# jean-pierreBoth/gsearch

Hardware: AMD Instinct MI355X
Metric: query genomes/sec (higher is better)
Workload: dtype f32

## Files before the change

### gsearch_amd/csrc/gs_join.hip

```cpp
#include <string.h>
#include <algorithm>
#include <chrono>
#include <vector>
#include "gs_internal.hpp"

namespace gs {

template <typename T> struct ElemKey;
template <> struct ElemKey<uint32_t> { static constexpr bool F = false; };

template <int KIND, typename T>
__device__ __forceinline__ T canon(T v)
{
    if (KIND == GS_KIND_F32) return (v == (T)0x80000000u) ? (T)0 : v;
    return v;
}
template <int KIND, typename T>
__device__ __forceinline__ bool never_equal(T v)
{
    if (KIND == GS_KIND_F32) return ((uint32_t)v & 0x7FFFFFFFu) > 0x7F800000u;
    return false;
}

template <typename T>
__global__ __launch_bounds__(256) void k_rows_to_cols(const uint8_t *__restrict__ rows, uint64_t stride, uint64_t nrows, uint32_t m, T *__restrict__ cols,
                                                       uint64_t colcap, uint64_t first, int f32)
{
    __shared__ T tile[32][33];
    const uint32_t tx = threadIdx.x & 31, ty = threadIdx.x >> 5;
    const uint64_t r0 = (uint64_t)blockIdx.x * 32, s0 = (uint64_t)blockIdx.y * 32;
    for (uint32_t j = ty; j < 32; j += 8) {
        const uint64_t r = r0 + j, s = s0 + tx;
        tile[j][tx] = (r < nrows && s < m) ? ((const T *)(rows + r * stride))[s] : (T)0;
    }
    __syncthreads();
    for (uint32_t j = ty; j < 32; j += 8) {
        const uint64_t s = s0 + j, r = r0 + tx;
        if (s < m && r < nrows) { const T v = tile[tx][j]; cols[s * colcap + first + r] = (f32 && v == (T)0x80000000u) ? (T)0 : v; }
    }
}

template <int KIND, typename T>
__global__ __launch_bounds__(256) void k_query_cols(const uint8_t *__restrict__ rows, uint64_t stride, uint32_t nq, uint32_t m, T *__restrict__ qkey)
{
    __shared__ T tile[32][33];
    const uint32_t tx = threadIdx.x & 31, ty = threadIdx.x >> 5;
    const uint64_t r0 = (uint64_t)blockIdx.x * 32, s0 = (uint64_t)blockIdx.y * 32;
    for (uint32_t j = ty; j < 32; j += 8) {
        const uint64_t r = r0 + j, s = s0 + tx;
        tile[j][tx] = (r < nq && s < m) ? ((const T *)(rows + r * stride))[s] : (T)0;
    }
    __syncthreads();
    for (uint32_t j = ty; j < 32; j += 8) {
        const uint64_t s = s0 + j, r = r0 + tx;
        if (s < m && r < nq) qkey[s * nq + r] = tile[tx][j];
    }
}

constexpr int JT = 1024;
constexpr int JU = 4;
constexpr int JP_MAX_LOG2 = 13;
constexpr int JQ_MAX = 3276;
constexpr int JB_LOG2 = 16;
constexpr uint32_t HTILE = 128;

__device__ __forceinline__ uint32_t join_hash(uint32_t k) { return k * 0x9E3779B1u; }
__device__ __forceinline__ uint32_t join_hash(uint64_t k) { return (uint32_t)((k * 0x9E3779B97F4A7C15ull) >> 32); }
#define GS_SEL4(a, i) (((i) & 2) ? (((i) & 1) ? a[3] : a[2]) : (((i) & 1) ? a[1] : a[0]))

#ifndef GS_JOIN_COUNT_KIND
#define GS_JOIN_COUNT_KIND 0
#endif
constexpr int JN = 8;
__device__ __forceinline__ void join_lds_barrier()
{
    __builtin_amdgcn_fence(__ATOMIC_RELEASE, "workgroup", "local");
    __builtin_amdgcn_s_barrier();
    __builtin_amdgcn_fence(__ATOMIC_ACQUIRE, "workgroup", "local");
}

__device__ __forceinline__ void join_wave_sync()
{
    __builtin_amdgcn_fence(__ATOMIC_RELEASE, "wavefront");
    __builtin_amdgcn_wave_barrier();
    __builtin_amdgcn_fence(__ATOMIC_ACQUIRE, "wavefront");
}

#define GS_JOIN_HIT(st, tagv, e)                                                                              \
    do {                                                                                                      \
        if (((st) & 0xFFFu) == (tagv)) (st) += 0x1000u;                                                       \
        else if ((st) < 0x2000u) { if (st) { join_flush(mm32, ld, (st), (e)); natom++; } (st) = (tagv) | 0x1000u; } \
        else { join_flush(mm32, ld, (tagv) | 0x1000u, (e)); natom++; }                                        \
    } while (0)
__device__ __forceinline__ void join_flush(uint32_t *mm32, uint64_t ld, uint32_t st, uint64_t e)
{
    const uint64_t idx = (uint64_t)((st & 0xFFFu) - 1) * ld + e;
    atomicSub(&mm32[idx >> 1], (st >> 12) << ((idx & 1) * 16));
}

constexpr uint32_t JTAG_MASK = 0xFFFu, JTAG_MULTI = 0x1000u, JTAG_MORE = 0x80000000u;
constexpr int JTAG_CL_SHIFT = 13;
constexpr uint32_t JCL_MAX = 2047;
constexpr int JWALK = 4;

template <int KIND, typename T, int SR, bool CL>
__global__ __launch_bounds__(JT, (sizeof(T) == 8 && SR == 1) ? 4 : 8) void k_match_join(const T *__restrict__ qkey, uint32_t nq, uint32_t log2p, const T *__restrict__ cols, uint64_t colcap, uint64_t n,
                                                    uint32_t slot_lo, uint32_t slot_hi, uint32_t slots_per_wg, uint32_t *__restrict__ mm32, uint64_t ld,
                                                    unsigned long long *__restrict__ stats, int chunk_major, uint64_t col0, const uint16_t *__restrict__ qcl,
                                                    const uint16_t *__restrict__ nodelab, const T *__restrict__ qs, uint32_t nh, const uint32_t *__restrict__ cl_lo,
                                                    const uint32_t *__restrict__ qlist, uint32_t dedup_flags)
{
    const uint32_t dedup_below = dedup_flags & 0x7FFFFFFFu;
    static_assert(JU == 4 && JN % JU == 0, "GS_SEL4 / pending mask are written for JU = 4");
    static_assert(!CL || SR == 1, "clusters: request batches only");
    constexpr bool E8 = sizeof(T) == 4 && SR == 1;
    constexpr bool DEDUP = CL && E8;
    constexpr bool D64 = sizeof(T) == 8 && SR == 1 && !CL;
    constexpr bool DENSE = E8 || D64;
    extern __shared__ __attribute__((aligned(16))) uint8_t s_raw[];
    const uint32_t P = 1u << log2p, mask = P - 1, sh = 32 - log2p;
    constexpr uint32_t BMW = (1u << JB_LOG2) / 32;
    uint32_t *tag = (uint32_t *)s_raw;
    uint32_t *bm = E8 ? (uint32_t *)(s_raw + 8 * (size_t)P) : (uint32_t *)(s_raw + 4 * (size_t)P * SR);
    T *key = (T *)(s_raw + (4 * (size_t)P + (size_t)BMW * 4) * SR);
    unsigned long long *ent = (unsigned long long *)s_raw;
    const uint32_t bchunk = chunk_major ? blockIdx.y : blockIdx.x, bslot = chunk_major ? blockIdx.x : blockIdx.y;
    const uint64_t e0 = (uint64_t)bchunk * (JT * JN) + threadIdx.x;
    const uint32_t s0 = slot_lo + bslot * slots_per_wg, s1 = s0 + slots_per_wg < slot_hi ? s0 + slots_per_wg : slot_hi;
    const uint2 *labT = CL ? (const uint2 *)nodelab + (uint64_t)bchunk * (JN / JU) * JT : nullptr;
    uint32_t sticky[JN];
    uint32_t natom = 0;
    uint32_t nexp = 0;
#pragma unroll
    for (int i = 0; i < JN; i++) sticky[i] = 0;
    const uint32_t lane = threadIdx.x & 63;
    uint32_t vmask = 0;
#pragma unroll
    for (int u = 0; u < JN; u++) vmask |= (uint32_t)(e0 + (uint64_t)u * JT < n) << u;
    const uint64_t ebase_u = col0 + (uint64_t)bchunk * (JT * JN);
    const uint32_t tid = threadIdx.x;
    uint32_t labmask = 0;
    if (CL && DENSE) {
#pragma unroll
        for (int it = 0; it < JN / JU; it++) {
            const uint2 l4 = labT[it * JT + threadIdx.x];
            labmask |= ((uint32_t)((l4.x & 0xFFFFu) != 0u) | (uint32_t)((l4.x >> 16) != 0u) << 1 | (uint32_t)((l4.y & 0xFFFFu) != 0u) << 2 | (uint32_t)((l4.y >> 16) != 0u) << 3) << (it * JU);
        }
    }
    const bool wave_lab = CL && DENSE && (dedup_flags >> 31) && __any(labmask != 0u);
    uint2 *wq = (uint2 *)(s_raw + (D64 ? 12 : 8) * (size_t)P + (size_t)BMW * 4) + (threadIdx.x >> 6) * (D64 ? 128 : 64);
    T vn[DENSE ? JN : JU];
#pragma unroll
    for (int u = 0; u < (DENSE ? JN : JU); u++) { const uint64_t e = e0 + (uint64_t)u * JT; vn[u] = (e < n && s0 < s1) ? cols[(uint64_t)s0 * colcap + e] : (T)0; }
    for (uint32_t sr = s0; sr < s1; sr += SR) {
        const uint32_t nr = s1 - sr < (uint32_t)SR ? s1 - sr : (uint32_t)SR;
        constexpr int JQ = DENSE ? (int)((((1u << JP_MAX_LOG2) * 2) / 5 + JT - 1) / JT) : 1;
        T kq[JQ];
        uint32_t tq[(JQ + 1) / 2] = {};
        if (DENSE) {
            typedef const T __attribute__((address_space(1))) *gptr;
            const uint64_t qb = (uint64_t)(qkey + (uint64_t)sr * nq);
            const gptr qk = (gptr)(((uint64_t)(uint32_t)__builtin_amdgcn_readfirstlane((uint32_t)(qb >> 32)) << 32) | (uint64_t)(uint32_t)__builtin_amdgcn_readfirstlane((uint32_t)qb));
            uint32_t o = threadIdx.x;
            asm volatile("" : "+v"(o));
#pragma unroll
            for (int j = 0; j < JQ; j++) { const gptr qj = qk + j * JT; kq[j] = o + (uint32_t)j * JT < nq ? qj[o] : (T)0; }
            if constexpr (CL) {
#pragma unroll
                for (int j = 0; j < JQ; j++) { const uint32_t i = o + (uint32_t)j * JT; tq[j >> 1] |= (i < nq ? (uint32_t)qcl[i] : 0u) << ((j & 1) * 16); }
            }
        }
        join_lds_barrier();
        if (E8) { for (uint32_t i = threadIdx.x; i < P; i += JT) ent[i] = 0ull; }
        else for (uint32_t i = threadIdx.x; i < P * SR; i += JT) tag[i] = 0;
        for (uint32_t i = threadIdx.x; i < BMW * SR; i += JT) bm[i] = 0;
        join_lds_barrier();
        auto insert_key = [&](const uint32_t r, const uint32_t q, T k, const uint32_t clq) {
            const uint32_t tw = CL ? (q + 1) | (clq << JTAG_CL_SHIFT) : q + 1;
            if (never_equal<KIND, T>(k)) return;
            k = canon<KIND, T>(k);
            const uint32_t hq = join_hash(k);
            atomicOr(&bm[r * BMW + (hq >> (32 - JB_LOG2 + 5))], (1u << ((hq >> (32 - JB_LOG2)) & 31)) | (1u << ((hq >> (27 - JB_LOG2)) & 31)));
            uint32_t h = hq >> sh;
            if (E8) {
                const unsigned long long nw = ((unsigned long long)tw << 32) | (uint32_t)k;
                for (;;) {
                    const unsigned long long old = atomicCAS(&ent[h], 0ull, nw);
                    if (old == 0ull) break;
                    if (DEDUP && (tw >> JTAG_CL_SHIFT) - 1u < dedup_below - 1u && (uint32_t)old == (uint32_t)k &&
                        (((uint32_t)(old >> 32) >> JTAG_CL_SHIFT) & JCL_MAX) == (tw >> JTAG_CL_SHIFT)) {
                        atomicOr((uint32_t *)&ent[h] + 1, JTAG_MULTI);
                        break;
                    }
                    if ((uint32_t)old == (uint32_t)k && !((uint32_t)(old >> 32) & JTAG_MORE)) atomicOr((uint32_t *)&ent[h] + 1, JTAG_MORE);
                    h = (h + 1) & mask;
                }
            } else {
                while (atomicCAS(&tag[r * P + h], 0u, tw) != 0u) h = (h + 1) & mask;
                key[r * P + h] = k;
            }
        };
        if (DENSE) {
#pragma unroll
            for (int j = 0; j < JQ; j++) { const uint32_t i = threadIdx.x + (uint32_t)j * JT; if (i < nq) insert_key(0u, i, kq[j], (tq[j >> 1] >> ((j & 1) * 16)) & 0xFFFFu); }
        } else {
            for (uint32_t i = threadIdx.x; i < nq * nr; i += JT) { const uint32_t r = i / nq, q = i - r * nq; insert_key(r, q, qkey[(uint64_t)(sr + r) * nq + q], CL ? (uint32_t)qcl[q] : 0u); }
        }
        uint2 lb0 = make_uint2(0u, 0u), lb1 = make_uint2(0u, 0u);
        if constexpr (CL && DENSE) {
            if (wave_lab) { uint32_t o0 = threadIdx.x, o1 = JT + threadIdx.x; asm volatile("" : "+v"(o0), "+v"(o1)); lb0 = labT[o0]; lb1 = labT[o1]; }
        }
        join_lds_barrier();
#pragma unroll 1
        for (uint32_t r = 0; r < nr; r++) {
            const uint32_t s = sr + r, tb = r * P, bb = r * BMW;
            const T *col = cols + (uint64_t)s * colcap;
            if constexpr (DENSE) {
                uint32_t pend = 0;
#pragma unroll
                for (int u0 = 0; u0 < JN; u0 += 4) {
                    uint32_t hsd[4], bwd[4];
#pragma unroll
                    for (int u = 0; u < 4; u++) { hsd[u] = join_hash(vn[u0 + u]); bwd[u] = bm[hsd[u] >> (32 - JB_LOG2 + 5)]; }
#pragma unroll
                    for (int u = 0; u < 4; u++) {
                        const uint32_t pass = (vmask >> (u0 + u)) & (bwd[u] >> ((hsd[u] >> (32 - JB_LOG2)) & 31)) & (bwd[u] >> ((hsd[u] >> (27 - JB_LOG2)) & 31)) & 1u;
                        pend |= pass << (u0 + u);
                    }
                }
                if constexpr (CL) {
                    if (wave_lab) {
#pragma unroll
                        for (int u = 0; u < JN; u++) {
                            const uint32_t l2 = u < 4 ? ((u & 2) ? lb0.y : lb0.x) : ((u & 2) ? lb1.y : lb1.x);
                            const uint32_t lab = (l2 >> ((u & 1) * 16)) & 0xFFFFu;
                            if (((pend >> u) & 1u) && lab != 0u) {
                                uint32_t hh = join_hash(vn[u]) >> sh;
#pragma unroll
                                for (int j = 0; j < JWALK; j++) {
                                    const unsigned long long en = ent[hh];
                                    const uint32_t t = (uint32_t)(en >> 32);
                                    if (t == 0u) { pend &= ~(1u << u); natom += GS_JOIN_COUNT_KIND == 8; break; }
                                    if ((uint32_t)en == (uint32_t)vn[u]) {
                                        if (((t >> JTAG_CL_SHIFT) & JCL_MAX) != lab) break;
                                        if (!(t & JTAG_MORE)) { pend &= ~(1u << u); natom += GS_JOIN_COUNT_KIND == 8; break; }
                                    }
                                    hh = (hh + 1) & mask;
                                }
                            }
                        }
                    }
                }
                while (__any(pend != 0u)) {
                    uint32_t qn = 0;
                    const uint32_t pend0 = pend;
#pragma unroll
                    for (int u = 0; u < JN; u++) {
                        const bool want = (pend >> u) & 1u;
                        const unsigned long long mw = __ballot(want);
                        const uint32_t cw = (uint32_t)__popcll(mw);
                        if (cw != 0u && qn + cw <= 64u) {
                            if (want) {
                                const uint32_t at = qn + __builtin_amdgcn_mbcnt_hi((uint32_t)(mw >> 32), __builtin_amdgcn_mbcnt_lo((uint32_t)mw, 0u));
                                const uint32_t who = lane | ((uint32_t)u << 6) | (sticky[u] << 9) | (CL ? ((labmask >> u) & 1u) << 29 : 0u);
                                if constexpr (D64) { wq[2 * at] = make_uint2((uint32_t)vn[u], (uint32_t)((uint64_t)vn[u] >> 32)); wq[2 * at + 1].x = who; }
                                else wq[at] = make_uint2((uint32_t)vn[u], who);
                            }
                            qn += cw; pend &= ~(1u << u);
                        }
                    }
                    join_wave_sync();
                    if constexpr (CL) {
                        if (GS_JOIN_COUNT_KIND == 7 && lane < qn) natom++;
                        bool have = lane < qn;
                        uint2 qe = make_uint2(0u, 0u);
                        if (have) qe = wq[lane];
                        uint32_t st = (qe.y >> 9) & 0xFFFFFu, flp = 0;
                        const uint32_t eloc = (qe.y & 63u) + ((qe.y >> 6) & 7u) * JT;
                        uint32_t hh = join_hash((T)qe.x) >> sh;
                        for (;;) {
                            uint32_t mitem = 0;
                            if (have) {
                                const unsigned long long en = ent[hh];
                                const uint32_t t = (uint32_t)(en >> 32);
                                if (t == 0u) have = false;
                                else {
                                    if ((uint32_t)en == qe.x) {
                                        if (!(t & JTAG_MORE)) have = false;
                                        bool count_it = true;
// ... 249 lines not shown
    __shared__ uint2 stage[HS_STAGE];
    __shared__ uint32_t sn;
    __shared__ unsigned long long sbase;
    if (threadIdx.x == 0) sn = 0;
    __syncthreads();
    const uint64_t tiles_per_row = (n + 2047) / 2048, ntiles = tiles_per_row * nq;
    uint32_t tot = 0;
    auto flush = [&]() {
        __syncthreads();
        const uint32_t cnt = sn;
        if (cnt) {
            if (threadIdx.x == 0) sbase = atomicAdd(&ctr[0], (unsigned long long)cnt);
            __syncthreads();
            const unsigned long long base = sbase;
            for (uint32_t i = threadIdx.x; i < cnt; i += 256) if (base + i < cap) pairs[base + i] = stage[i];
            __syncthreads();
            if (threadIdx.x == 0) sn = 0;
        }
        __syncthreads();
    };
    for (uint64_t t = blockIdx.x; t < ntiles; t += gridDim.x) {
        const uint32_t q = (uint32_t)(t / tiles_per_row);
        const uint64_t e8 = (t - (uint64_t)q * tiles_per_row) * 2048 + (uint64_t)threadIdx.x * 8;
        if (e8 < n) {
            const uint4 w = *(const uint4 *)(mat + (uint64_t)q * ld + e8);
            const uint32_t ww[4] = {w.x, w.y, w.z, w.w};
#pragma unroll
            for (int i = 0; i < 8; i++) {
                const uint32_t c = (ww[i >> 1] >> ((i & 1) * 16)) & 0xFFFFu;
                const uint32_t def = (e8 + i < n) ? m - c : 0u;
                tot += def;
                if (def >= JHEAVY) stage[atomicAdd(&sn, 1u)] = make_uint2((uint32_t)(e8 + i), q | (def << 16));
            }
        }
        __syncthreads();
        if (sn >= HS_STAGE - 2048) flush();
    }
    flush();
#pragma unroll
    for (int o = 32; o > 0; o >>= 1) tot += __shfl_down(tot, o);
    if ((threadIdx.x & 63) == 0 && tot) atomicAdd(&ctr[1], (unsigned long long)tot);
}
__global__ void k_label_init(uint32_t *__restrict__ labq, uint32_t nq, uint32_t *__restrict__ labe, uint64_t n)
{
    const uint64_t i = (uint64_t)blockIdx.x * blockDim.x + threadIdx.x;
    if (i < nq) labq[i] = (uint32_t)i;
    if (i < n) labe[i] = 0xFFFFFFFFu;
}
__global__ void k_label_prop(const uint2 *__restrict__ pairs, const unsigned long long *__restrict__ ctr, uint64_t cap, uint32_t *__restrict__ labq, uint32_t *__restrict__ labe)
{
    const uint64_t np = ctr[0] < cap ? ctr[0] : cap;
    for (uint64_t i = (uint64_t)blockIdx.x * blockDim.x + threadIdx.x; i < np; i += (uint64_t)gridDim.x * blockDim.x) {
        const uint2 p = pairs[i];
        const uint32_t q = p.y & 0xFFFFu, a = labq[q], b = labe[p.x], l = a < b ? a : b;
        if (l < a) atomicMin(&labq[q], l);
        if (l < b) atomicMin(&labe[p.x], l);
    }
}
__global__ void k_label_count(const uint32_t *__restrict__ labe, uint64_t n, uint32_t nq, uint32_t *__restrict__ cnt)
{
    for (uint64_t e = (uint64_t)blockIdx.x * blockDim.x + threadIdx.x; e < n; e += (uint64_t)gridDim.x * blockDim.x) { const uint32_t l = labe[e]; if (l < nq) atomicAdd(&cnt[l], 1u); }
}
template <typename T>
__global__ __launch_bounds__(256) void k_query_cols_list(const uint8_t *__restrict__ rows, uint64_t stride, const uint32_t *__restrict__ qlist, uint32_t nh, uint32_t m, T *__restrict__ qs)
{
    __shared__ T tile[32][33];
    const uint32_t tx = threadIdx.x & 31, ty = threadIdx.x >> 5;
    const uint64_t r0 = (uint64_t)blockIdx.x * 32, s0 = (uint64_t)blockIdx.y * 32;
    for (uint32_t j = ty; j < 32; j += 8) {
        const uint64_t r = r0 + j, s = s0 + tx;
        tile[j][tx] = (r < nh && s < m) ? ((const T *)(rows + (uint64_t)qlist[r] * stride))[s] : (T)0;
    }
    __syncthreads();
    for (uint32_t j = ty; j < 32; j += 8) {
        const uint64_t s = s0 + j, r = r0 + tx;
        if (s < m && r < nh) qs[s * nh + r] = tile[tx][j];
    }
}
struct JoinGeom { uint32_t chunks, log2p; size_t lds1, ldsq; };

template <int KIND, typename T, bool CL>
static int join_launch(gs_ctx *c, const JoinGeom &g, const T *qkey, uint32_t nq, const void *cols, uint64_t colcap, uint64_t n, uint32_t slot_lo, uint32_t slot_hi,
                       uint16_t *out16, uint64_t ld, unsigned long long *stats, uint64_t col0, bool few_blocks, const uint16_t *qcl, const uint16_t *nodelab, const T *qs,
                       uint32_t nh, const uint32_t *cl_lo, const uint32_t *qlist, uint32_t dedup_below = 0)
{
    const uint32_t ms = slot_hi - slot_lo, chunks = g.chunks;
    uint32_t blocks = std::max<uint32_t>(1, std::min<uint32_t>((16 * c->n_cu) / chunks, std::max<uint32_t>(ms / 32, (2 * c->n_cu) / chunks)));
    if (few_blocks) blocks = std::max<uint32_t>(1, std::min<uint32_t>(ms / 4, (2 * c->n_cu + chunks - 1) / chunks));
    if (getenv("GS_JOIN_BLOCKS") && !few_blocks) blocks = (uint32_t)atoi(getenv("GS_JOIN_BLOCKS"));
    blocks = std::min<uint32_t>(std::max<uint32_t>(blocks, 1), ms);
    const uint32_t slots_per_wg = (ms + blocks - 1) / blocks;
    const int chunk_major = getenv("GS_JOIN_CHUNK_MAJOR") ? atoi(getenv("GS_JOIN_CHUNK_MAJOR")) : ((nq >= 1024 && chunks >= 16) ? 1 : 0);
    const uint32_t nblk = (ms + slots_per_wg - 1) / slots_per_wg;
    dim3 jg(chunk_major ? nblk : chunks, chunk_major ? chunks : nblk);
    int sr = 1;
    if (!CL) {
        if (4 * g.lds1 <= 80 * 1024 && slots_per_wg >= 8) sr = 4; else if (2 * g.lds1 <= 80 * 1024 && slots_per_wg >= 4) sr = 2;
        if (getenv("GS_JOIN_SLOTS_PER_ROUND")) { const int e = atoi(getenv("GS_JOIN_SLOTS_PER_ROUND")); if (e == 1 || (e == 2 && 2 * g.lds1 <= 80 * 1024) || (e == 4 && 4 * g.lds1 <= 80 * 1024)) sr = e; }
    }
    const size_t lds = g.lds1 * sr + (sr == 1 ? g.ldsq : 0);
    ProfScope ps(c, FAM_HAMMING);
#define GS_JOIN_GO(KERN)                                                                                                                              \
    do {                                                                                                                                              \
        auto kern = KERN;                                                                                                                             \
        if (lds > 48 * 1024) GS_HIP_CHECK(hipFuncSetAttribute((const void *)kern, hipFuncAttributeMaxDynamicSharedMemorySize, (int)lds));             \
        hipLaunchKernelGGL(kern, jg, dim3(JT), lds, c->stream, qkey, nq, g.log2p, (const T *)cols, colcap, n, slot_lo, slot_hi, slots_per_wg, (uint32_t *)out16, ld, \
                           stats, chunk_major, col0, qcl, nodelab, qs, nh, cl_lo, qlist, dedup_below);                                                             \
    } while (0)
    if (CL) GS_JOIN_GO((k_match_join<KIND, T, 1, CL>));
    else if (sr == 4) GS_JOIN_GO((k_match_join<KIND, T, 4, false>));
    else if (sr == 2) GS_JOIN_GO((k_match_join<KIND, T, 2, false>));
    else GS_JOIN_GO((k_match_join<KIND, T, 1, false>));
#undef GS_JOIN_GO
    GS_HIP_CHECK(hipGetLastError());
    return GS_OK;
}

template <int KIND, typename T>
static int join_sample_declines(gs_ctx *c, const JoinGeom &g, uint32_t m, const T *qkey, uint32_t nq, const void *cols, uint64_t colcap, uint64_t n, DevBuf *scratch, int *decline_out)
{
    int rc;
    const uint32_t nsamp = 24;
    DevBuf &cnt = scratch[1];
    if ((rc = cnt.ensure(16))) return rc;
    GS_HIP_CHECK(hipMemsetAsync(cnt.p, 0, 16, c->stream));
    const size_t lds_s = (sizeof(T) + 4) * ((size_t)1 << g.log2p);
    auto ks = k_match_sample<KIND, T>;
    if (lds_s > 48 * 1024) GS_HIP_CHECK(hipFuncSetAttribute((const void *)ks, hipFuncAttributeMaxDynamicSharedMemorySize, (int)lds_s));
    hipLaunchKernelGGL(ks, dim3(g.chunks, nsamp), dim3(JT), lds_s, c->stream, qkey, nq, g.log2p, (const T *)cols, colcap, n, m, nsamp, cnt.as<unsigned long long>());
    GS_HIP_CHECK(hipGetLastError());
    unsigned long long hr[2] = {0, 0};
    GS_HIP_CHECK(hipMemcpyAsync(hr, cnt.p, 16, hipMemcpyDeviceToHost, c->stream));
    GS_HIP_CHECK(hipStreamSynchronize(c->stream));
    const double scale = (double)m / (double)nsamp;
    const double atomics = (double)(hr[0] - hr[1]) * scale + (double)hr[1] * scale / 64.0;
    const double t_join = (double)n * m * sizeof(T) / 3.5e12 + atomics / 1.6e10 + (double)hr[0] * scale / 2.0e11;
    const double t_tile = (double)((nq + 127) / 128 * 128) * (double)n * (double)m / (KIND == GS_KIND_U64 ? 1.4e13 : 1.6e13);
    const char *force = getenv("GS_JOIN_DECLINE");
    const bool decline = force ? atoi(force) != 0 : t_join > t_tile;
    if (getenv("GS_JOIN_VERBOSE"))
        fprintf(stderr, "[GS_JOIN] nq=%u n=%llu sampled matches %llu repeats %llu -> est. join %.2f ms, tile %.2f ms: %s\n", nq, (unsigned long long)n, hr[0], hr[1],
                t_join * 1e3, t_tile * 1e3, decline ? "tile" : "join");
    *decline_out = decline ? 1 : 0;
    return GS_OK;
}

template <int KIND, typename T>
static int join_impl(gs_ctx *c, uint32_t m, const uint8_t *qrows, uint64_t qstride, uint32_t nq, const void *cols, uint64_t colcap, uint64_t n, uint16_t *out16,
                     uint64_t ld, DevBuf *scratch , int *declined, unsigned long long *stats, bool init, uint64_t col0,
                     const void *rows, uint64_t rstride)
{
    int rc;
    if (declined) *declined = 0;
    const size_t items = (size_t)m * nq;
    DevBuf &k0 = scratch[0];
    if ((rc = k0.ensure(sizeof(T) * items))) return rc;
    if (init) GS_HIP_CHECK(hipMemsetD16Async((hipDeviceptr_t)out16, (unsigned short)m, (size_t)nq * ld, c->stream));
    dim3 tg((nq + 31) / 32, (m + 31) / 32);
    hipLaunchKernelGGL((k_query_cols<KIND, T>), tg, dim3(256), 0, c->stream, qrows, qstride, nq, m, k0.as<T>());
    GS_HIP_CHECK(hipGetLastError());
    JoinGeom g;
    g.log2p = 6;
    while (g.log2p < (uint32_t)JP_MAX_LOG2 && (double)(1u << g.log2p) * 0.4 < (double)nq) g.log2p++;
    g.chunks = (uint32_t)((n + (uint64_t)JT * JN - 1) / ((uint64_t)JT * JN));
    g.lds1 = (sizeof(T) + 4) * ((size_t)1 << g.log2p) + ((size_t)1 << JB_LOG2) / 8;
    g.ldsq = (size_t)(JT / 64) * 64 * (sizeof(T) == 4 ? 8 : 16);
    const bool may_decline = declined && m >= 64 && n >= 4096;
    const char *ce = getenv("GS_JOIN_CLUSTER");
    bool cluster = declined && init && col0 == 0 && rows && nq >= 256 && n >= 8192 && m >= 16 * JS0 && (ld % 8) == 0 && !(ce && !atoi(ce)) && !getenv("GS_JOIN_DECLINE");
    if (ce && atoi(ce) == 2) cluster = declined && init && col0 == 0 && rows && m >= 2 * JS0 && (ld % 8) == 0;
    if (!cluster) {
        if (may_decline) {
            int dec = 0;
            if ((rc = join_sample_declines<KIND, T>(c, g, m, k0.as<T>(), nq, cols, colcap, n, scratch, &dec))) return rc;
            if (dec) { *declined = 1; return GS_OK; }
        }
        return join_launch<KIND, T, false>(c, g, k0.as<T>(), nq, cols, colcap, n, 0, m, out16, ld, stats, col0, false, nullptr, nullptr, nullptr, 0, nullptr, nullptr);
    }
    const bool verbose = getenv("GS_JOIN_VERBOSE") != nullptr;
    const bool times = getenv("GS_JOIN_TIMES") != nullptr;
    auto t_prev = std::chrono::steady_clock::now();
    auto lap = [&](const char *what) {
        if (!times) return;
        (void)hipStreamSynchronize(c->stream);
        const auto now = std::chrono::steady_clock::now();
        fprintf(stderr, "[GS_JOIN_TIMES] %-28s %8.3f ms\n", what, std::chrono::duration<double, std::milli>(now - t_prev).count());
        t_prev = now;
    };
    lap("query columns + memset");
    DevBuf &pairs = scratch[2], &ctr = scratch[3], &labq = scratch[4], &labe = scratch[5];
    uint64_t pair_cap = JPAIR_CAP;
    DevBuf &lcnt = scratch[14];
    if ((rc = pairs.ensure(pair_cap * 8)) || (rc = ctr.ensure(64)) || (rc = labq.ensure(4 * (size_t)nq)) || (rc = labe.ensure(4 * (size_t)n)) || (rc = lcnt.ensure(4 * (size_t)nq))) return rc;
    pair_cap = std::max<uint64_t>(pair_cap, pairs.bytes / 8);
    if ((rc = join_launch<KIND, T, false>(c, g, k0.as<T>(), nq, cols, colcap, n, 0, JS0, out16, ld, stats, 0, true, nullptr, nullptr, nullptr, 0, nullptr, nullptr))) return rc;
    lap("phase 0 (first slots)");
    uint8_t *pin = (uint8_t *)pinned_pool(c)->ensure(PIN_JOIN, 64 + 4 * (2 * (size_t)nq + n) + 2 * ((size_t)nq + 8 + (size_t)g.chunks * JT * JN) + 64);
    GS_REQUIRE(pin, GS_ERR_HIP, "match-join: pinned staging buffer");
    unsigned long long *hc = (unsigned long long *)pin;
    uint32_t *hlq = (uint32_t *)(pin + 64), *hcn = hlq + nq, *hle = hcn + nq;
    for (int attempt = 0;; attempt++) {
        GS_HIP_CHECK(hipMemsetAsync(ctr.p, 0, 64, c->stream));
        hipLaunchKernelGGL(k_heavy_scan, dim3(c->n_cu * 8), dim3(256), 0, c->stream, out16, ld, nq, n, m, pairs.as<uint2>(), ctr.as<unsigned long long>(), pair_cap);
        lap("heavy scan");
        hipLaunchKernelGGL(k_label_init, dim3((uint32_t)((std::max<uint64_t>(n, nq) + 255) / 256)), dim3(256), 0, c->stream, labq.as<uint32_t>(), nq, labe.as<uint32_t>(), n);
        for (int it = 0; it < 6; it++)
            hipLaunchKernelGGL(k_label_prop, dim3(c->n_cu * 4), dim3(256), 0, c->stream, pairs.as<uint2>(), ctr.as<unsigned long long>(), pair_cap, labq.as<uint32_t>(), labe.as<uint32_t>());
        GS_HIP_CHECK(hipMemsetAsync(lcnt.p, 0, 4 * (size_t)nq, c->stream));
        hipLaunchKernelGGL(k_label_count, dim3(c->n_cu * 2), dim3(256), 0, c->stream, labe.as<uint32_t>(), n, nq, lcnt.as<uint32_t>());
        GS_HIP_CHECK(hipGetLastError());
        GS_HIP_CHECK(hipMemcpyAsync(hc, ctr.p, 16, hipMemcpyDeviceToHost, c->stream));
        GS_HIP_CHECK(hipMemcpyAsync(hlq, labq.p, 4 * (size_t)nq, hipMemcpyDeviceToHost, c->stream));
        GS_HIP_CHECK(hipMemcpyAsync(hcn, lcnt.p, 4 * (size_t)nq, hipMemcpyDeviceToHost, c->stream));
        GS_HIP_CHECK(hipStreamSynchronize(c->stream));
        lap("labels + query labels down");
        if (hc[0] <= pair_cap || attempt || hc[0] > JPAIR_MAX) break;
        if (pairs.alloc((size_t)hc[0] * 8 + 4096) != GS_OK) { (void)hipGetLastError(); (void)pairs.alloc(JPAIR_CAP * 8); pair_cap = JPAIR_CAP; break; }
        pair_cap = hc[0] + 512;
    }
    const uint64_t npairs = hc[0];
    std::vector<uint32_t> cq(nq, 0), ce_(nq, 0), cid(nq, 0);
    uint32_t K = 0, ntiles = 0, nhq = 0, dedup_below = 1;
    uint64_t nhe = 0;
    const uint32_t minq = getenv("GS_JOIN_CLUSTER_MINQ") ? (uint32_t)std::max(2, atoi(getenv("GS_JOIN_CLUSTER_MINQ"))) : (ce && atoi(ce) == 2 ? 2u : 12u);
    const uint64_t minpairs = getenv("GS_JOIN_CLUSTER_MINPAIRS") ? (uint64_t)atoll(getenv("GS_JOIN_CLUSTER_MINPAIRS")) : 128;
    auto is_cluster = [&](uint32_t l) { return cq[l] >= minq || (cq[l] >= 2 && (uint64_t)(cq[l] - 1) * hcn[l] >= minpairs); };
    const uint64_t min_scaled0 = (uint64_t)((double)nq * 32.0 * (double)n / 3.0e5);
    const uint64_t min_saved0 = getenv("GS_JOIN_CLUSTER_MIN") ? (uint64_t)atoll(getenv("GS_JOIN_CLUSTER_MIN")) : (ce && atoi(ce) == 2 ? 0 : std::max<uint64_t>((uint64_t)nq * 8, min_scaled0));
    bool any = false;
    if (npairs <= pair_cap) {
        for (uint32_t q = 0; q < nq; q++) if (hlq[q] < nq) ++cq[hlq[q]];
        uint64_t est = 0;
        for (uint32_t l = 0; l < nq; l++) if (cq[l] && hcn[l] && is_cluster(l)) { any = true; est += (uint64_t)(cq[l] - 1) * hcn[l]; }
        if (est < min_saved0) any = false;
    }
    if (any) {
        GS_HIP_CHECK(hipMemcpyAsync(hle, labe.p, 4 * (size_t)n, hipMemcpyDeviceToHost, c->stream));
        GS_HIP_CHECK(hipStreamSynchronize(c->stream));
        for (uint64_t e = 0; e < n; e++) if (hle[e] < nq) ce_[hle[e]]++;
        std::vector<uint32_t> order;
        for (uint32_t l = 0; l < nq; l++) if (ce_[l] >= 1 && is_cluster(l)) order.push_back(l);
        auto tiles_of = [&](uint32_t l) { return ((cq[l] + HTILE - 1) / HTILE) * ((ce_[l] + HTILE - 1) / HTILE); };
        std::sort(order.begin(), order.end(), [&](uint32_t a, uint32_t b) { const uint32_t ta = tiles_of(a), tb = tiles_of(b); return ta != tb ? ta < tb : a < b; });
        std::vector<uint32_t> chosen;
        for (uint32_t l : order) {
            if (chosen.size() >= JCL_MAX || ntiles + tiles_of(l) > JTILE_CAP) break;
            chosen.push_back(l); ntiles += tiles_of(l); nhq += cq[l]; nhe += ce_[l];
        }
        const uint32_t dq = getenv("GS_JOIN_DEDUP_MINQ") ? (uint32_t)std::max(2, atoi(getenv("GS_JOIN_DEDUP_MINQ"))) : JDEDUP_MINQ;
        std::stable_sort(chosen.begin(), chosen.end(), [&](uint32_t a, uint32_t b) { return (cq[a] >= dq) > (cq[b] >= dq); });
        for (uint32_t l : chosen) { cid[l] = ++K; if (cq[l] >= dq) dedup_below = K + 1; }
    }
    uint64_t saved_pairs = 0;
    for (uint32_t l = 0; l < nq; l++) if (cid[l]) saved_pairs += (uint64_t)(cq[l] - 1) * ce_[l];
    const uint64_t min_scaled = (uint64_t)((double)nq * 32.0 * (double)n / 3.0e5);
    const uint64_t min_saved = getenv("GS_JOIN_CLUSTER_MIN") ? (uint64_t)atoll(getenv("GS_JOIN_CLUSTER_MIN")) : (ce && atoi(ce) == 2 ? 0 : std::max<uint64_t>((uint64_t)nq * 8, min_scaled));
    if (verbose)
        fprintf(stderr, "[GS_JOIN] nq=%u n=%llu heavy pairs %llu (matches in the first %u slots %llu): %u clusters, %u queries x %llu nodes in %u tiles, %llu pairs off the atomics%s\n", nq,
                (unsigned long long)n, (unsigned long long)npairs, JS0, hc[1], K, nhq, (unsigned long long)nhe, ntiles, (unsigned long long)saved_pairs,
                K && saved_pairs < min_saved ? " - not worth the cluster-aware pass" : "");
    if (K && saved_pairs < min_saved) K = 0;
    lap("host: components");
    if (K == 0) {
        const double t_tile = (double)((nq + 127) / 128 * 128) * (double)n * (double)m / (KIND == GS_KIND_U64 ? 1.4e13 : 1.6e13);
        if (may_decline && (npairs > pair_cap || (double)hc[1] * ((double)m / JS0) / 1.6e10 > 0.5 * t_tile)) {
            int dec = 0;
            if ((rc = join_sample_declines<KIND, T>(c, g, m, k0.as<T>(), nq, cols, colcap, n, scratch, &dec))) return rc;
            if (dec) { *declined = 1; return GS_OK; }
        }
        return join_launch<KIND, T, false>(c, g, k0.as<T>(), nq, cols, colcap, n, JS0, m, out16, ld, stats, 0, false, nullptr, nullptr, nullptr, 0, nullptr, nullptr);
    }
    std::vector<uint32_t> cl_lo(K + 2, 0), ce_lo(K + 2, 0);
    for (uint32_t l = 0; l < nq; l++) if (cid[l]) { cl_lo[cid[l] + 1] = cq[l]; ce_lo[cid[l] + 1] = ce_[l]; }
    for (uint32_t k = 1; k <= K + 1; k++) { cl_lo[k] += cl_lo[k - 1]; ce_lo[k] += ce_lo[k - 1]; }
    std::vector<uint32_t> qlist(nhq), elist(nhe), fq(cl_lo.begin(), cl_lo.end()), fe(ce_lo.begin(), ce_lo.end());
    const uint64_t npad = (uint64_t)g.chunks * JT * JN;
    uint16_t *hqcl = (uint16_t *)(hle + n), *hnl = hqcl + ((nq + 3) & ~3u);
    for (uint32_t q = 0; q < nq; q++) { const uint32_t l = hlq[q]; hqcl[q] = 0; if (l < nq && cid[l]) { hqcl[q] = (uint16_t)cid[l]; qlist[fq[cid[l]]++] = q; } }
    memset(hnl, 0, 2 * npad);
    for (uint64_t e = 0; e < n; e++) {
        const uint32_t l = hle[e];
        if (l < nq && cid[l]) {
            const uint64_t ch = e / (JT * JN), w = e % (JT * JN), i = w / JT, ln = w % JT;
            hnl[((ch * (JN / JU) + i / JU) * JT + ln) * JU + i % JU] = (uint16_t)cid[l];
            elist[fe[cid[l]]++] = (uint32_t)e;
        }
    }
    std::vector<uint4> tiles;
    tiles.reserve(ntiles);
    uint32_t n_thin = 0;
    for (int pass = 0; pass < 2; pass++)
        for (uint32_t k = 1; k <= K; k++)
            for (uint32_t a = cl_lo[k]; a < cl_lo[k + 1]; a += HTILE) {
                const uint32_t qr = std::min<uint32_t>(HTILE, cl_lo[k + 1] - a);
                if ((qr <= 16) != (pass == 0)) continue;
                for (uint32_t b = ce_lo[k]; b < ce_lo[k + 1]; b += HTILE) {
                    tiles.push_back(make_uint4(a, qr, b, std::min<uint32_t>(HTILE, ce_lo[k + 1] - b)));
                    n_thin += pass == 0;
                }
            }
    lap("host: lists");
    DevBuf &dqcl = scratch[6], &dnl = scratch[7], &dql = scratch[8], &del = scratch[9], &dtl = scratch[10], &dqs = scratch[11], &dcl = scratch[13];
    if ((rc = dqcl.ensure(2 * (size_t)nq)) || (rc = dnl.ensure(2 * (size_t)npad)) || (rc = dql.ensure(4 * (size_t)nhq)) || (rc = del.ensure(4 * (size_t)nhe)) ||
        (rc = dtl.ensure(16 * tiles.size())) || (rc = dqs.ensure(sizeof(T) * (size_t)m * nhq)) || (rc = dcl.ensure(4 * (size_t)(K + 2)))) return rc;
    GS_HIP_CHECK(hipMemcpyAsync(dqcl.p, hqcl, 2 * (size_t)nq, hipMemcpyHostToDevice, c->stream));
    GS_HIP_CHECK(hipMemcpyAsync(dnl.p, hnl, 2 * (size_t)npad, hipMemcpyHostToDevice, c->stream));
    GS_HIP_CHECK(hipMemcpyAsync(dql.p, qlist.data(), 4 * (size_t)nhq, hipMemcpyHostToDevice, c->stream));
    GS_HIP_CHECK(hipMemcpyAsync(del.p, elist.data(), 4 * (size_t)nhe, hipMemcpyHostToDevice, c->stream));
    GS_HIP_CHECK(hipMemcpyAsync(dtl.p, tiles.data(), 16 * tiles.size(), hipMemcpyHostToDevice, c->stream));
    GS_HIP_CHECK(hipMemcpyAsync(dcl.p, cl_lo.data(), 4 * (size_t)(K + 2), hipMemcpyHostToDevice, c->stream));
    GS_HIP_CHECK(hipStreamSynchronize(c->stream));
    hipLaunchKernelGGL((k_query_cols_list<T>), dim3((nhq + 31) / 32, (m + 31) / 32), dim3(256), 0, c->stream, qrows, qstride, dql.as<uint32_t>(), nhq, m, dqs.as<T>());
    GS_HIP_CHECK(hipGetLastError());
    lap("uploads + sorted key copy");
    const bool inplace = getenv("GS_JOIN_INPLACE") ? atoi(getenv("GS_JOIN_INPLACE")) != 0 : nhe * 10 >= n;
    if ((rc = join_launch<KIND, T, true>(c, g, k0.as<T>(), nq, cols, colcap, n, JS0, m, out16, ld, stats, 0, false, dqcl.as<uint16_t>(), dnl.as<uint16_t>(), dqs.as<T>(), nhq,
                                         dcl.as<uint32_t>(), dql.as<uint32_t>(), dedup_below | (inplace ? 0x80000000u : 0u)))) return rc;
    {
        ProfScope ps(c, FAM_HAMMING);
        lap("cluster-aware join");
        if ((rc = hamming_blocks(c, KIND, m, qrows, qstride, rows, rstride, dtl.p, (uint32_t)tiles.size(), dql.as<uint32_t>(), del.as<uint32_t>(), out16, ld, n_thin))) return rc;
        lap("block compare");
    }
    return GS_OK;
}

uint64_t match_join_max_queries() { const char *e = getenv("GS_JOIN_MAXQ"); return e ? (uint64_t)std::max(1, std::min(4094, atoi(e))) : JQ_MAX; }

int match_join_counts(gs_ctx *c, int kind, uint32_t m, const void *qrows, uint64_t qstride, uint64_t nq, const void *cols, uint64_t colcap, uint64_t n,
                      uint16_t *out16, uint64_t ld, DevBuf *scratch, int *declined, unsigned long long *stats, bool init, uint64_t col0, const void *rows, uint64_t rstride)
{
    GS_REQUIRE(nq >= 1 && nq <= 4094 && m <= 65535 && (ld % 2) == 0 && ((uintptr_t)out16 % 4) == 0, GS_ERR_INVALID, "match_join_counts: bad shape");
    GS_REQUIRE((uint64_t)m * nq < ((uint64_t)1 << 31), GS_ERR_INVALID, "match_join_counts: batch too large");
    if (kind == GS_KIND_U64) return join_impl<GS_KIND_U64, uint64_t>(c, m, (const uint8_t *)qrows, qstride, (uint32_t)nq, cols, colcap, n, out16, ld, scratch, declined, stats, init, col0, rows, rstride);
    if (kind == GS_KIND_F32) return join_impl<GS_KIND_F32, uint32_t>(c, m, (const uint8_t *)qrows, qstride, (uint32_t)nq, cols, colcap, n, out16, ld, scratch, declined, stats, init, col0, rows, rstride);
    return join_impl<GS_KIND_U32, uint32_t>(c, m, (const uint8_t *)qrows, qstride, (uint32_t)nq, cols, colcap, n, out16, ld, scratch, declined, stats, init, col0, rows, rstride);
}

int rows_to_cols(gs_ctx *c, int kind, uint32_t m, const void *rows, uint64_t stride, uint64_t nrows, void *cols, uint64_t colcap, uint64_t first)
{
    if (nrows == 0) return GS_OK;
    dim3 g((uint32_t)((nrows + 31) / 32), (m + 31) / 32);
    if (kind == GS_KIND_U64) hipLaunchKernelGGL((k_rows_to_cols<uint64_t>), g, dim3(256), 0, c->stream, (const uint8_t *)rows, stride, nrows, m, (uint64_t *)cols, colcap, first, 0);
    else hipLaunchKernelGGL((k_rows_to_cols<uint32_t>), g, dim3(256), 0, c->stream, (const uint8_t *)rows, stride, nrows, m, (uint32_t *)cols, colcap, first, (int)(kind == GS_KIND_F32));
    GS_HIP_CHECK(hipGetLastError());
    return GS_OK;
}

}
```

Measured before the change: 48390.

## Prebuild per-slot LDS hash table images once, load them in join

Adds a prepass kernel that builds each slot's query hash table and bloom bitmap once, then writes a compact image of entry positions and bitmap words to global memory. The f32 join kernel then loads these images and places entries directly into LDS instead of redoing atomic CAS inserts in every workgroup that shares the slot. This removes redundant per-chunk table construction and its atomic contention. The cost is an extra kernel launch, a global image buffer of slots×nq×8 bytes plus bitmaps, and extra global reads per slot.

```diff
diff --git a/gsearch_amd/csrc/gs_join.hip b/gsearch_amd/csrc/gs_join.hip
--- a/gsearch_amd/csrc/gs_join.hip
+++ b/gsearch_amd/csrc/gs_join.hip
@@ -103,18 +103,81 @@
 constexpr uint32_t JCL_MAX = 2047;
 constexpr int JWALK = 4;
 
+constexpr int JQ4 = (int)((((1u << JP_MAX_LOG2) * 2) / 5 + JT - 1) / JT);
+constexpr uint32_t JIMG_POS_HI = 1u << 24, JIMG_VALID = 1u << 25, JIMG_NONE = 0xFFFFFFFFu;
+constexpr uint32_t JIMG_TAG_KEEP = JTAG_MORE | JTAG_MULTI | (JCL_MAX << JTAG_CL_SHIFT);
+static_assert(JQ4 == 4 && JP_MAX_LOG2 == 13 && (JIMG_TAG_KEEP & (JTAG_MASK | JIMG_POS_HI | JIMG_VALID)) == 0, "image layout");
+static_assert((1u << JB_LOG2) / 32 == 2 * JT, "a lane copies two bitmap words");
+
+template <int KIND, bool CL>
+__device__ __forceinline__ uint32_t join_insert8(unsigned long long *ent, uint32_t *bm, uint32_t mask, uint32_t sh, uint32_t k, uint32_t q, uint32_t clq, uint32_t dedup_below)
+{
+    const uint32_t tw = CL ? (q + 1) | (clq << JTAG_CL_SHIFT) : q + 1;
+    if (never_equal<KIND, uint32_t>(k)) return JIMG_NONE;
+    k = canon<KIND, uint32_t>(k);
+    const uint32_t hq = join_hash(k);
+    atomicOr(&bm[hq >> (32 - JB_LOG2 + 5)], (1u << ((hq >> (32 - JB_LOG2)) & 31)) | (1u << ((hq >> (27 - JB_LOG2)) & 31)));
+    uint32_t h = hq >> sh;
+    const unsigned long long nw = ((unsigned long long)tw << 32) | k;
+    for (;;) {
+        const unsigned long long old = atomicCAS(&ent[h], 0ull, nw);
+        if (old == 0ull) return h;
+        if (CL && (tw >> JTAG_CL_SHIFT) - 1u < dedup_below - 1u && (uint32_t)old == k && (((uint32_t)(old >> 32) >> JTAG_CL_SHIFT) & JCL_MAX) == (tw >> JTAG_CL_SHIFT)) {
+            atomicOr((uint32_t *)&ent[h] + 1, JTAG_MULTI);
+            return JIMG_NONE;
+        }
+        if ((uint32_t)old == k && !((uint32_t)(old >> 32) & JTAG_MORE)) atomicOr((uint32_t *)&ent[h] + 1, JTAG_MORE);
+        h = (h + 1) & mask;
+    }
+}
+
+template <int KIND, bool CL>
+__global__ __launch_bounds__(JT) void k_join_tables(const uint32_t *__restrict__ qkey, uint32_t nq, uint32_t log2p, uint32_t slot_lo, const uint16_t *__restrict__ qcl, uint32_t dedup_below,
+                                                     unsigned long long *__restrict__ img_e, uint32_t *__restrict__ img_b)
+{
+    extern __shared__ __attribute__((aligned(16))) uint8_t s_raw[];
+    const uint32_t P = 1u << log2p, mask = P - 1, sh = 32 - log2p;
+    constexpr uint32_t BMW = (1u << JB_LOG2) / 32;
+    unsigned long long *ent = (unsigned long long *)s_raw;
+    uint32_t *bm = (uint32_t *)(s_raw + 8 * (size_t)P);
+    const uint32_t b = blockIdx.x;
+    const uint32_t *qk = qkey + (uint64_t)(slot_lo + b) * nq;
+    for (uint32_t i = threadIdx.x; i < P; i += JT) ent[i] = 0ull;
+    for (uint32_t i = threadIdx.x; i < BMW; i += JT) bm[i] = 0;
+    __syncthreads();
+    uint32_t at[JQ4];
+#pragma unroll
+    for (int j = 0; j < JQ4; j++) {
+        const uint32_t q = threadIdx.x + (uint32_t)j * JT;
+        at[j] = q < nq ? join_insert8<KIND, CL>(ent, bm, mask, sh, qk[q], q, CL ? (uint32_t)qcl[q] : 0u, dedup_below) : JIMG_NONE;
+    }
+    __syncthreads();
+#pragma unroll
+    for (int j = 0; j < JQ4; j++) {
+        const uint32_t q = threadIdx.x + (uint32_t)j * JT;
+        if (q < nq) {
+            unsigned long long e = 0ull;
+            if (at[j] != JIMG_NONE) {
+                const unsigned long long f = ent[at[j]];
+                e = (unsigned long long)(((uint32_t)(f >> 32) & JIMG_TAG_KEEP) | (at[j] & JTAG_MASK) | ((at[j] >> 12) << 24) | JIMG_VALID) << 32 | (uint32_t)f;
+            }
+            img_e[(uint64_t)b * nq + q] = e;
+        }
+    }
+    for (uint32_t i = threadIdx.x; i < BMW; i += JT) img_b[(uint64_t)b * BMW + i] = bm[i];
+}
+
 template <int KIND, typename T, int SR, bool CL>
 __global__ __launch_bounds__(JT, (sizeof(T) == 8 && SR == 1) ? 4 : 8) void k_match_join(const T *__restrict__ qkey, uint32_t nq, uint32_t log2p, const T *__restrict__ cols, uint64_t colcap, uint64_t n,
                                                     uint32_t slot_lo, uint32_t slot_hi, uint32_t slots_per_wg, uint32_t *__restrict__ mm32, uint64_t ld,
                                                     unsigned long long *__restrict__ stats, int chunk_major, uint64_t col0, const uint16_t *__restrict__ qcl,
                                                     const uint16_t *__restrict__ nodelab, const T *__restrict__ qs, uint32_t nh, const uint32_t *__restrict__ cl_lo,
-                                                    const uint32_t *__restrict__ qlist, uint32_t dedup_flags)
-{
-    const uint32_t dedup_below = dedup_flags & 0x7FFFFFFFu;
+                                                    const uint32_t *__restrict__ qlist, uint32_t dedup_flags, const unsigned long long *__restrict__ img_e,
+                                                    const uint32_t *__restrict__ img_b)
+{
     static_assert(JU == 4 && JN % JU == 0, "GS_SEL4 / pending mask are written for JU = 4");
     static_assert(!CL || SR == 1, "clusters: request batches only");
     constexpr bool E8 = sizeof(T) == 4 && SR == 1;
-    constexpr bool DEDUP = CL && E8;
     constexpr bool D64 = sizeof(T) == 8 && SR == 1 && !CL;
     constexpr bool DENSE = E8 || D64;
     extern __shared__ __attribute__((aligned(16))) uint8_t s_raw[];
@@ -154,10 +217,23 @@
     for (int u = 0; u < (DENSE ? JN : JU); u++) { const uint64_t e = e0 + (uint64_t)u * JT; vn[u] = (e < n && s0 < s1) ? cols[(uint64_t)s0 * colcap + e] : (T)0; }
     for (uint32_t sr = s0; sr < s1; sr += SR) {
         const uint32_t nr = s1 - sr < (uint32_t)SR ? s1 - sr : (uint32_t)SR;
-        constexpr int JQ = DENSE ? (int)((((1u << JP_MAX_LOG2) * 2) / 5 + JT - 1) / JT) : 1;
-        T kq[JQ];
-        uint32_t tq[(JQ + 1) / 2] = {};
-        if (DENSE) {
+        constexpr int JQ = DENSE ? JQ4 : 1;
+        T kq[E8 ? 1 : JQ];
+        unsigned long long ie[E8 ? JQ : 1];
+        unsigned long long ib = 0ull;
+        uint32_t o8 = 0;
+        if constexpr (E8) {
+            typedef const uint8_t __attribute__((address_space(1))) *gptr1;
+            typedef const unsigned long long __attribute__((address_space(1))) *gptr8;
+            const uint64_t qb = (uint64_t)(img_e + (uint64_t)(sr - slot_lo) * nq), bb = (uint64_t)((const uint2 *)img_b + (uint64_t)(sr - slot_lo) * JT);
+            const gptr1 qk = (gptr1)(((uint64_t)(uint32_t)__builtin_amdgcn_readfirstlane((uint32_t)(qb >> 32)) << 32) | (uint64_t)(uint32_t)__builtin_amdgcn_readfirstlane((uint32_t)qb));
+            const gptr1 bk = (gptr1)(((uint64_t)(uint32_t)__builtin_amdgcn_readfirstlane((uint32_t)(bb >> 32)) << 32) | (uint64_t)(uint32_t)__builtin_amdgcn_readfirstlane((uint32_t)bb));
+            o8 = threadIdx.x * 8u;
+            asm volatile("" : "+v"(o8));
+#pragma unroll
+            for (int j = 0; j < JQ; j++) ie[j] = threadIdx.x + (uint32_t)j * JT < nq ? *(gptr8)(qk + j * JT * 8 + o8) : 0ull;
+            ib = *(gptr8)(bk + o8);
+        } else if constexpr (DENSE) {
             typedef const T __attribute__((address_space(1))) *gptr;
             const uint64_t qb = (uint64_t)(qkey + (uint64_t)sr * nq);
             const gptr qk = (gptr)(((uint64_t)(uint32_t)__builtin_amdgcn_readfirstlane((uint32_t)(qb >> 32)) << 32) | (uint64_t)(uint32_t)__builtin_amdgcn_readfirstlane((uint32_t)qb));
@@ -165,46 +241,42 @@
             asm volatile("" : "+v"(o));
 #pragma unroll
             for (int j = 0; j < JQ; j++) { const gptr qj = qk + j * JT; kq[j] = o + (uint32_t)j * JT < nq ? qj[o] : (T)0; }
-            if constexpr (CL) {
-#pragma unroll
-                for (int j = 0; j < JQ; j++) { const uint32_t i = o + (uint32_t)j * JT; tq[j >> 1] |= (i < nq ? (uint32_t)qcl[i] : 0u) << ((j & 1) * 16); }
+        }
+        join_lds_barrier();
+        if constexpr (E8) {
+            if (log2p == (uint32_t)JP_MAX_LOG2) {
+#pragma unroll
+                for (int k = 0; k < 4; k++) *(uint4 *)(s_raw + k * 16 * JT + 2 * o8) = make_uint4(0u, 0u, 0u, 0u);
+            } else
+                for (uint32_t i = o8; i < 8 * P; i += 8 * JT) *(unsigned long long *)(s_raw + i) = 0ull;
+            join_lds_barrier();
+            *(unsigned long long *)((uint8_t *)bm + o8) = ib;
+#pragma unroll
+            for (int j = 0; j < JQ; j++) {
+                const uint32_t w = (uint32_t)(ie[j] >> 32);
+                if (w != 0u)
+                    ent[((w & JTAG_MASK) | ((w >> 12) & 0x1000u)) & mask] = (unsigned long long)((w & JIMG_TAG_KEEP) | (tid + (uint32_t)j * JT + 1u)) << 32 | (uint32_t)ie[j];
             }
-        }
-        join_lds_barrier();
-        if (E8) { for (uint32_t i = threadIdx.x; i < P; i += JT) ent[i] = 0ull; }
-        else for (uint32_t i = threadIdx.x; i < P * SR; i += JT) tag[i] = 0;
-        for (uint32_t i = threadIdx.x; i < BMW * SR; i += JT) bm[i] = 0;
-        join_lds_barrier();
-        auto insert_key = [&](const uint32_t r, const uint32_t q, T k, const uint32_t clq) {
-            const uint32_t tw = CL ? (q + 1) | (clq << JTAG_CL_SHIFT) : q + 1;
-            if (never_equal<KIND, T>(k)) return;
-            k = canon<KIND, T>(k);
-            const uint32_t hq = join_hash(k);
-            atomicOr(&bm[r * BMW + (hq >> (32 - JB_LOG2 + 5))], (1u << ((hq >> (32 - JB_LOG2)) & 31)) | (1u << ((hq >> (27 - JB_LOG2)) & 31)));
-            uint32_t h = hq >> sh;
-            if (E8) {
-                const unsigned long long nw = ((unsigned long long)tw << 32) | (uint32_t)k;
-                for (;;) {
-                    const unsigned long long old = atomicCAS(&ent[h], 0ull, nw);
-                    if (old == 0ull) break;
-                    if (DEDUP && (tw >> JTAG_CL_SHIFT) - 1u < dedup_below - 1u && (uint32_t)old == (uint32_t)k &&
-                        (((uint32_t)(old >> 32) >> JTAG_CL_SHIFT) & JCL_MAX) == (tw >> JTAG_CL_SHIFT)) {
-                        atomicOr((uint32_t *)&ent[h] + 1, JTAG_MULTI);
-                        break;
-                    }
-                    if ((uint32_t)old == (uint32_t)k && !((uint32_t)(old >> 32) & JTAG_MORE)) atomicOr((uint32_t *)&ent[h] + 1, JTAG_MORE);
-                    h = (h + 1) & mask;
-                }
-            } else {
+        } else {
+            for (uint32_t i = threadIdx.x; i < P * SR; i += JT) tag[i] = 0;
+            for (uint32_t i = threadIdx.x; i < BMW * SR; i += JT) bm[i] = 0;
+            join_lds_barrier();
+            auto insert_key = [&](const uint32_t r, const uint32_t q, T k, const uint32_t clq) {
+                const uint32_t tw = CL ? (q + 1) | (clq << JTAG_CL_SHIFT) : q + 1;
+                if (never_equal<KIND, T>(k)) return;
+                k = canon<KIND, T>(k);
+                const uint32_t hq = join_hash(k);
+                atomicOr(&bm[r * BMW + (hq >> (32 - JB_LOG2 + 5))], (1u << ((hq >> (32 - JB_LOG2)) & 31)) | (1u << ((hq >> (27 - JB_LOG2)) & 31)));
+                uint32_t h = hq >> sh;
                 while (atomicCAS(&tag[r * P + h], 0u, tw) != 0u) h = (h + 1) & mask;
                 key[r * P + h] = k;
+            };
+            if (DENSE) {
+#pragma unroll
+                for (int j = 0; j < JQ; j++) { const uint32_t i = threadIdx.x + (uint32_t)j * JT; if (i < nq) insert_key(0u, i, kq[j], 0u); }
+            } else {
+                for (uint32_t i = threadIdx.x; i < nq * nr; i += JT) { const uint32_t r = i / nq, q = i - r * nq; insert_key(r, q, qkey[(uint64_t)(sr + r) * nq + q], CL ? (uint32_t)qcl[q] : 0u); }
             }
-        };
-        if (DENSE) {
-#pragma unroll
-            for (int j = 0; j < JQ; j++) { const uint32_t i = threadIdx.x + (uint32_t)j * JT; if (i < nq) insert_key(0u, i, kq[j], (tq[j >> 1] >> ((j & 1) * 16)) & 0xFFFFu); }
-        } else {
-            for (uint32_t i = threadIdx.x; i < nq * nr; i += JT) { const uint32_t r = i / nq, q = i - r * nq; insert_key(r, q, qkey[(uint64_t)(sr + r) * nq + q], CL ? (uint32_t)qcl[q] : 0u); }
         }
         uint2 lb0 = make_uint2(0u, 0u), lb1 = make_uint2(0u, 0u);
         if constexpr (CL && DENSE) {
@@ -620,7 +692,7 @@
 template <int KIND, typename T, bool CL>
 static int join_launch(gs_ctx *c, const JoinGeom &g, const T *qkey, uint32_t nq, const void *cols, uint64_t colcap, uint64_t n, uint32_t slot_lo, uint32_t slot_hi,
                        uint16_t *out16, uint64_t ld, unsigned long long *stats, uint64_t col0, bool few_blocks, const uint16_t *qcl, const uint16_t *nodelab, const T *qs,
-                       uint32_t nh, const uint32_t *cl_lo, const uint32_t *qlist, uint32_t dedup_below = 0)
+                       uint32_t nh, const uint32_t *cl_lo, const uint32_t *qlist, DevBuf &img, uint32_t dedup_below = 0)
 {
     const uint32_t ms = slot_hi - slot_lo, chunks = g.chunks;
     uint32_t blocks = std::max<uint32_t>(1, std::min<uint32_t>((16 * c->n_cu) / chunks, std::max<uint32_t>(ms / 32, (2 * c->n_cu) / chunks)));
@@ -638,12 +710,28 @@
     }
     const size_t lds = g.lds1 * sr + (sr == 1 ? g.ldsq : 0);
     ProfScope ps(c, FAM_HAMMING);
-#define GS_JOIN_GO(KERN)                                                                                                                              \
+    const unsigned long long *img_e = nullptr;
+    const uint32_t *img_b = nullptr;
+    if constexpr (sizeof(T) == 4) {
+        if (sr == 1) {
+            const size_t be = ((size_t)ms * nq * 8 + 15) & ~(size_t)15, bb = (size_t)ms * (((size_t)1 << JB_LOG2) / 8);
+            int rc;
+            if ((rc = img.ensure(be + bb))) return rc;
+            uint8_t *ib = img.as<uint8_t>();
+            img_e = (const unsigned long long *)ib; img_b = (const uint32_t *)(ib + be);
+            auto kt = k_join_tables<KIND, CL>;
+            if (g.lds1 > 48 * 1024) GS_HIP_CHECK(hipFuncSetAttribute((const void *)kt, hipFuncAttributeMaxDynamicSharedMemorySize, (int)g.lds1));
+            hipLaunchKernelGGL(kt, dim3(ms), dim3(JT), g.lds1, c->stream, (const uint32_t *)qkey, nq, g.log2p, slot_lo, qcl, dedup_below & 0x7FFFFFFFu, (unsigned long long *)img_e,
+                               (uint32_t *)img_b);
+            GS_HIP_CHECK(hipGetLastError());
+        }
+    }
+#define GS_JOIN_GO(KERN)                                                                                                                            \
     do {                                                                                                                                              \
         auto kern = KERN;                                                                                                                             \
         if (lds > 48 * 1024) GS_HIP_CHECK(hipFuncSetAttribute((const void *)kern, hipFuncAttributeMaxDynamicSharedMemorySize, (int)lds));             \
         hipLaunchKernelGGL(kern, jg, dim3(JT), lds, c->stream, qkey, nq, g.log2p, (const T *)cols, colcap, n, slot_lo, slot_hi, slots_per_wg, (uint32_t *)out16, ld, \
-                           stats, chunk_major, col0, qcl, nodelab, qs, nh, cl_lo, qlist, dedup_below);                                                             \
+                           stats, chunk_major, col0, qcl, nodelab, qs, nh, cl_lo, qlist, dedup_below, img_e, img_b);                                                                    \
     } while (0)
     if (CL) GS_JOIN_GO((k_match_join<KIND, T, 1, CL>));
     else if (sr == 4) GS_JOIN_GO((k_match_join<KIND, T, 4, false>));
@@ -713,7 +801,7 @@
             if ((rc = join_sample_declines<KIND, T>(c, g, m, k0.as<T>(), nq, cols, colcap, n, scratch, &dec))) return rc;
             if (dec) { *declined = 1; return GS_OK; }
         }
-        return join_launch<KIND, T, false>(c, g, k0.as<T>(), nq, cols, colcap, n, 0, m, out16, ld, stats, col0, false, nullptr, nullptr, nullptr, 0, nullptr, nullptr);
+        return join_launch<KIND, T, false>(c, g, k0.as<T>(), nq, cols, colcap, n, 0, m, out16, ld, stats, col0, false, nullptr, nullptr, nullptr, 0, nullptr, nullptr, scratch[12]);
     }
     const bool verbose = getenv("GS_JOIN_VERBOSE") != nullptr;
     const bool times = getenv("GS_JOIN_TIMES") != nullptr;
@@ -731,7 +819,7 @@
     DevBuf &lcnt = scratch[14];
     if ((rc = pairs.ensure(pair_cap * 8)) || (rc = ctr.ensure(64)) || (rc = labq.ensure(4 * (size_t)nq)) || (rc = labe.ensure(4 * (size_t)n)) || (rc = lcnt.ensure(4 * (size_t)nq))) return rc;
     pair_cap = std::max<uint64_t>(pair_cap, pairs.bytes / 8);
-    if ((rc = join_launch<KIND, T, false>(c, g, k0.as<T>(), nq, cols, colcap, n, 0, JS0, out16, ld, stats, 0, true, nullptr, nullptr, nullptr, 0, nullptr, nullptr))) return rc;
+    if ((rc = join_launch<KIND, T, false>(c, g, k0.as<T>(), nq, cols, colcap, n, 0, JS0, out16, ld, stats, 0, true, nullptr, nullptr, nullptr, 0, nullptr, nullptr, scratch[12]))) return rc;
     lap("phase 0 (first slots)");
     uint8_t *pin = (uint8_t *)pinned_pool(c)->ensure(PIN_JOIN, 64 + 4 * (2 * (size_t)nq + n) + 2 * ((size_t)nq + 8 + (size_t)g.chunks * JT * JN) + 64);
     GS_REQUIRE(pin, GS_ERR_HIP, "match-join: pinned staging buffer");
@@ -806,7 +894,7 @@
             if ((rc = join_sample_declines<KIND, T>(c, g, m, k0.as<T>(), nq, cols, colcap, n, scratch, &dec))) return rc;
             if (dec) { *declined = 1; return GS_OK; }
         }
-        return join_launch<KIND, T, false>(c, g, k0.as<T>(), nq, cols, colcap, n, JS0, m, out16, ld, stats, 0, false, nullptr, nullptr, nullptr, 0, nullptr, nullptr);
+        return join_launch<KIND, T, false>(c, g, k0.as<T>(), nq, cols, colcap, n, JS0, m, out16, ld, stats, 0, false, nullptr, nullptr, nullptr, 0, nullptr, nullptr, scratch[12]);
     }
     std::vector<uint32_t> cl_lo(K + 2, 0), ce_lo(K + 2, 0);
     for (uint32_t l = 0; l < nq; l++) if (cid[l]) { cl_lo[cid[l] + 1] = cq[l]; ce_lo[cid[l] + 1] = ce_[l]; }
@@ -853,7 +941,7 @@
     lap("uploads + sorted key copy");
     const bool inplace = getenv("GS_JOIN_INPLACE") ? atoi(getenv("GS_JOIN_INPLACE")) != 0 : nhe * 10 >= n;
     if ((rc = join_launch<KIND, T, true>(c, g, k0.as<T>(), nq, cols, colcap, n, JS0, m, out16, ld, stats, 0, false, dqcl.as<uint16_t>(), dnl.as<uint16_t>(), dqs.as<T>(), nhq,
-                                         dcl.as<uint32_t>(), dql.as<uint32_t>(), dedup_below | (inplace ? 0x80000000u : 0u)))) return rc;
+                                         dcl.as<uint32_t>(), dql.as<uint32_t>(), scratch[12], dedup_below | (inplace ? 0x80000000u : 0u)))) return rc;
     {
         ProfScope ps(c, FAM_HAMMING);
         lap("cluster-aware join");
```

Result: no change. 48250 (-0.3%).
